# duyhominhnguyen/conan-fgw

Hardware: AMD Instinct MI355X
Metric: molecules/s (K=5 conformers) (higher is better)
Workload: dtype f32

## Files before the change

### conan-fgw_amd/csrc/fgw_common.h

```cpp
#pragma once
#include <type_traits>
#include "common.h"

#ifdef CONAN_FGW_PROFILE
static __device__ long long g_fgw_prof[32];
#define FGW_PROF_ACCESSOR(name)                                                          \
    extern "C" int name(long long *out, int reset) {                                     \
        if (out && hipMemcpyFromSymbol(out, HIP_SYMBOL(g_fgw_prof), sizeof(long long) * 32) != hipSuccess) return -2; \
        if (reset) { long long z[32] = {0}; if (hipMemcpyToSymbol(HIP_SYMBOL(g_fgw_prof), z, sizeof(z)) != hipSuccess) return -2; } \
        return 0;                                                                        \
    }
static __device__ long long g_fgw_trace[2 + 6 * 8192];
#define FGW_PROF_TRACE_ACCESSOR(name)                                                    \
    extern "C" int name(long long *out, int reset) {                                     \
        if (out && hipMemcpyFromSymbol(out, HIP_SYMBOL(g_fgw_trace), sizeof(long long) * (2 + 6 * 8192)) != hipSuccess) return -2; \
        if (reset) { long long z[2] = {0, 0}; if (hipMemcpyToSymbol(HIP_SYMBOL(g_fgw_trace), z, sizeof(z)) != hipSuccess) return -2; } \
        return 0;                                                                        \
    }
#define FGW_PROF_TRACE(tag)                                                              \
    do {                                                                                 \
        if (threadIdx.x == 0) {                                                          \
            const unsigned long long i_ = atomicAdd(reinterpret_cast<unsigned long long *>(&g_fgw_trace[0]), 1ull); \
            if (i_ < 8192) {                                                             \
                long long *r_ = &g_fgw_trace[2 + 6 * i_];                                \
// ... 59 lines not shown
    int *order;
};
template <int NT>
__device__ __forceinline__ void adj_scatter_lds_bytes(const FgwAdj &A, int g, int N, int P, unsigned char *m, int tid) {
    const int lo = A.gptr[g], n = min(A.gptr[g + 1] - lo, N);
    const int e0 = A.rowptr[lo], e1 = A.rowptr[lo + n];
    for (int e = e0 + tid; e < e1; e += NT) {
        const int i = A.tgt[e] - lo, j = A.col[e] - lo;
        if (i >= 0 && i < N && j >= 0 && j < N) {
            const unsigned o = (unsigned)(j * P + i);
            atomicAdd(reinterpret_cast<unsigned *>(m + (o & ~3u)), 1u << (8 * (o & 3u)));
        }
    }
}
template <int NT>
__device__ __forceinline__ const float *adj_dense_slice(const FgwAdj &A, int g, int N, int tid) {
    float *dst = A.dense + (size_t)g * N * N;
    for (int t = tid; t < N * N; t += NT) dst[t] = 0.f;
    __syncthreads();
    const int lo = A.gptr[g], n = min(A.gptr[g + 1] - lo, N);
    const int e0 = A.rowptr[lo], e1 = A.rowptr[lo + n];
    for (int e = e0 + tid; e < e1; e += NT) {
        const int i = A.tgt[e] - lo, j = A.col[e] - lo;
        if (i >= 0 && i < N && j >= 0 && j < N) atomicAdd(&dst[j * N + i], 1.0f);
    }
    __threadfence_block();
    __syncthreads();
    return dst;
}

struct FastConst {
    double two_alpha, one_m_alpha, four_alpha_inv_eps, inv_eps, inner_tol, stop_thr, inv_n;
};
inline FastConst fast_const(const conan_fgw_params &prm, int N) {
    const double alpha = (double)prm.alpha, inv_eps = 1.0 / (double)prm.epsilon;
    return FastConst{2.0 * alpha, 1.0 - alpha, 4.0 * alpha * inv_eps, inv_eps, (double)prm.inner_tol, (double)prm.stop_thr, 1.0 / (double)N};
}

__device__ __forceinline__ double exp_acc(double x) {
    if (x < -745.0) return 0.0;
    const double t = x * 1.4426950408889634074;
    const double n = rint(t);
    const float f = (float)(t - n);
    const float e = __builtin_amdgcn_exp2f(f);
    return ldexp((double)e, (int)n);
}

__device__ __forceinline__ double exp_fast(double x) {
    const double xc = fmin(fmax(x, -700.0), 700.0);
    const double t = xc * 1.4426950408889634074;
    const double sh = t + 6755399441055744.0;
    const int n = __double2loint(sh);
    const double f = t - (sh - 6755399441055744.0);
    const double e = (double)__builtin_amdgcn_exp2f((float)f);
    const double scale = __hiloint2double((n + 1023) << 20, 0);
    const double r = e * scale;
    return x > -700.0 ? (x < 700.0 ? r : __builtin_inf()) : 0.0;
}

__device__ __forceinline__ double rcp_pos(double s) {
    double r = __builtin_amdgcn_rcp(s);
    r = fma(fma(-s, r, 1.0), r, r);
    r = fma(fma(-s, r, 1.0), r, r);
    return r;
}

__device__ __forceinline__ double log_acc(double s) {
    const double y0 = (double)(__builtin_amdgcn_logf((float)s) * 0.693147180559945309f);
    const double r = s * exp_acc(-y0) - 1.0;
    return y0 + (r - 0.5 * r * r);
}

__device__ __forceinline__ double wave_sum_d(double v) {
#pragma unroll
    for (int o = 32; o > 0; o >>= 1) v += __shfl_xor(v, o, 64);
    return v;
}
__device__ __forceinline__ double wave_max_d(double v) {
#pragma unroll
    for (int o = 32; o > 0; o >>= 1) { double w = __shfl_xor(v, o, 64); v = w > v ? w : v; }
    return v;
}

template <int NW = FGW_WAVES>
__device__ __forceinline__ double block_sum_d(double v, double *red) {
    v = wave_sum_d(v);
    __syncthreads();
    if ((threadIdx.x & 63) == 0) red[threadIdx.x >> 6] = v;
    __syncthreads();
    double s = 0.0;
#pragma unroll
    for (int w = 0; w < NW; ++w) s += red[w];
    return s;
}


typedef double f64x4 __attribute__((ext_vector_type(4)));

__device__ __forceinline__ double exp_lse(double x) {
    const float f = (float)x;
    return (double)__builtin_amdgcn_exp2f(f * 1.44269504088896340736f);
}

template <int NW = FGW_WAVES, class FX, class FW, class FS>
__device__ __forceinline__ void mm_f64_pad(int M, int Nn, int Kd, FX X, FW W, FS st) {
    const int lane = threadIdx.x & 63, wave = __builtin_amdgcn_readfirstlane((int)(threadIdx.x >> 6));
    const int Mq = (M + 15) >> 4, Nq = (Nn + 15) >> 4;
    const int li = lane & 15, lk = lane >> 4;
    for (int t = wave; t < Mq * Nq; t += NW) {
        const int i0 = (t / Nq) << 4, j0 = (t % Nq) << 4;
        const int ia = i0 + li, jb = j0 + li;
        const bool ra = ia < M, cb = jb < Nn;
        const int ic = ra ? ia : M - 1, jc = cb ? jb : Nn - 1;
        f64x4 acc = {0.0, 0.0, 0.0, 0.0};
        int k0 = 0;
        for (; k0 + 16 <= Kd; k0 += 16) {
            double a[4], b[4];
#pragma unroll
            for (int u = 0; u < 4; ++u) { a[u] = X(ic, k0 + 4 * u + lk); b[u] = W(k0 + 4 * u + lk, jc); }
#pragma unroll
            for (int u = 0; u < 4; ++u) acc = __builtin_amdgcn_mfma_f64_16x16x4f64(ra ? a[u] : 0.0, cb ? b[u] : 0.0, acc, 0, 0, 0);
        }
        if (k0 < Kd) {
            double a[4], b[4];
#pragma unroll
            for (int u = 0; u < 4; ++u) {
                const int k = k0 + 4 * u + lk, kc = k < Kd ? k : Kd - 1;
                a[u] = X(ic, kc); b[u] = W(kc, jc);
            }
#pragma unroll
            for (int u = 0; u < 4; ++u) {
                const bool kin = k0 + 4 * u + lk < Kd;
                if (k0 + 4 * u < Kd)
                    acc = __builtin_amdgcn_mfma_f64_16x16x4f64((ra && kin) ? a[u] : 0.0, (cb && kin) ? b[u] : 0.0, acc, 0, 0, 0);
            }
        }
#pragma unroll
        for (int q = 0; q < 4; ++q) {
            const int i = i0 + lk + 4 * q;
            if (i < M && cb) st(i, jb, acc[q]);
        }
    }
}

template <int NW, bool WT, typename TX, typename TW, class FS>
__device__ __forceinline__ void mm_f64_glb(int M, int Nn, int Kd, const TX *__restrict__ X, int pX, const TW *__restrict__ W, int pW, FS st,
                                           const int tid = threadIdx.x) {
    const int lane = tid & 63, wave = __builtin_amdgcn_readfirstlane(tid >> 6);
    const int Mq = (M + 15) >> 4, Nq = (Nn + 15) >> 4;
    const int li = lane & 15, lk = lane >> 4;
    for (int t = wave; t < Mq * Nq; t += NW) {
        const int i0 = (t / Nq) << 4, j0 = (t % Nq) << 4;
        const int ia = i0 + li, jb = j0 + li;
        const bool ra = ia < M, cb = jb < Nn;
        const TX *xr = X + (size_t)(ra ? ia : M - 1) * pX;
        const int jc = cb ? jb : Nn - 1;
        f64x4 acc = {0.0, 0.0, 0.0, 0.0}, acc2 = {0.0, 0.0, 0.0, 0.0};
        for (int k0 = 0; k0 < Kd; k0 += 16) {
            const int kb = k0 + 4 * lk;
            double a[4], b[4];
            if (k0 + 16 <= Kd) {
#pragma unroll
                for (int u = 0; u < 4; ++u) a[u] = (double)xr[kb + u];
                if (WT) {
                    const TW *wr = W + (size_t)jc * pW + kb;
#pragma unroll
                    for (int u = 0; u < 4; ++u) b[u] = (double)wr[u];
                } else {
#pragma unroll
                    for (int u = 0; u < 4; ++u) b[u] = (double)W[(size_t)(kb + u) * pW + jc];
                }
// ... 756 lines not shown
```

### conan-fgw_amd/csrc/fgw_small.hip

```cpp
#include "fgw_common.h"

#ifdef CONAN_FGW_PROFILE
FGW_PROF_ACCESSOR(conan_debug_fgw_prof)
FGW_PROF_TRACE_ACCESSOR(conan_debug_fgw_trace)
#endif

namespace {

constexpr int SK_SCRATCH_DOUBLES = 3 * 256 + 2 * 64;

template <int R, bool KL, bool SECOND = false>
__global__ void __launch_bounds__(FGW_THREADS, (SECOND || R > 9) ? 1 : 3) k_fgw_coupling_small(
    const float *__restrict__ Ys, const float *__restrict__ Cs, const float *__restrict__ ps, const float *__restrict__ pb,
    FgwDims D, conan_fgw_params prm, int outer, int y_zero, const double *__restrict__ Cw, const double *__restrict__ Yw,
    const int *__restrict__ active, float *__restrict__ Tw, int *__restrict__ info, fgw_part_t *__restrict__ Ypart,
    fgw_part_t *__restrict__ Cpart, const double *__restrict__ zvec, const double *__restrict__ yvec, const int *__restrict__ only, FgwAdj adj) {
    extern __shared__ __attribute__((aligned(16))) char smem[];
    auto solve = [&](const int cid) {
    const int b = cid / D.K, s = cid % D.K;
    if (!fgw_active(active, D.B, b, outer)) return;
    const int N = D.N, P = D.P, d = D.d;
    const int NN = N * N, NP = N * P;
    const int tid = threadIdx.x, lane = tid & 63, w = __builtin_amdgcn_readfirstlane(tid >> 6);
    const bool lane_ok = lane < N;
// ... 276 lines not shown

    if (!prm.fixed_features && Ypart) {
        fgw_part_t *Yp = Ypart + ((size_t)b * D.K + s) * N * d;
        if (z_lds) {
            const int Nd = N * d;
            for (int t0 = tid; t0 < Nd; t0 += 4 * FGW_THREADS) {
                float zv[4];
#pragma unroll
                for (int u = 0; u < 4; ++u) { const int t = t0 + u * FGW_THREADS; zv[u] = Z[t < Nd ? t : Nd - 1]; }
#pragma unroll
                for (int u = 0; u < 4; ++u) { const int t = t0 + u * FGW_THREADS; if (t < Nd) Zl2[t] = zv[u]; }
            }
            __syncthreads();
            mm_lds<FGW_WAVES, false>(N, d, N, Tl, P, Zl2, d, [&](int i, int c, double v) { Yp[(size_t)i * d + c] = (fgw_part_t)v; }, border_prepare(N, d));
        } else {
            mm_f64(N, d, N, [&](int i, int k) { return (double)Tl[i * P + k]; }, [&](int k, int c) { return (double)Z[(size_t)k * d + c]; },
                   [&](int i, int c, double v) { Yp[(size_t)i * d + c] = (fgw_part_t)v; });
        }
    }
    FGW_PROF(9);
    if (!prm.fixed_structure) {
        fgw_part_t *Cp = Cpart + ((size_t)b * D.K + s) * NN;
        if constexpr (KL)
            mm_f64(N, N, N, [&](int i, int k) { return (double)Tl[i * P + k]; },
                   [&](int k, int j) { const double cv = (double)C2l[k * P + j]; return log(cv > 1e-15 ? cv : 1e-15); },
                   [&](int i, int j, double v) { Al[i * P + j] = v; }, bnn);
        else
            mm_lds<FGW_WAVES, false>(N, N, N, Tl, P, C2l, P, [&](int i, int j, double v) { Al[i * P + j] = v; }, bnn);
        __syncthreads();
        mm_lds<FGW_WAVES, true>(N, N, N, Al, P, Tl, P, [&](int i, int j, double v) { Cp[i * N + j] = (fgw_part_t)v; }, bnn);
    }
    FGW_PROF(10);
    FGW_PROF_FLUSH;
    };
    if constexpr (!SECOND) solve(blockIdx.x);
    else {
        const int total = D.B * D.K, base = (int)blockIdx.x * 64, l = (int)threadIdx.x & 63;
        unsigned long long m = __ballot(base + l < total && only[base + l < total ? base + l : 0] != 0);
        while (m) {
            const int k = __ffsll((long long)m) - 1;
            m &= m - 1;
            solve(base + k);
            __syncthreads();
        }
    }
}

template <int R> struct FastCfg {
    static constexpr int OCC = R <= 9 ? 5 : (R <= 12 ? 2 : 1);
};
inline int fast_tiles_per_wave(int N) {
    const int Mc = (N >> 4) << 4;
    const bool border = (N - Mc) * N + Mc * (N - Mc) <= FGW_WAVES * 32 && Mc > 0;
    const int q = border ? N >> 4 : (N + 15) >> 4;
    return (q * q + FGW_WAVES - 1) / FGW_WAVES;
}
constexpr int FAST_VEC_DOUBLES = 128 + 256;
constexpr int FAST_SK_DOUBLES = 2 * 256 + 2 * 64;

struct FastLds {
    int npa;
    size_t off_t, off_c2, off_red, off_vec, off_sk, off_rs, bytes;
    bool vec_alias, sk_alias;
};
template <typename C2T>
__host__ __device__ inline FastLds fast_lds(int N) {
    FastLds L;
    const int NP = N * fgw_pitch(N);
    L.npa = (NP + 1) & ~1;
    size_t o = (size_t)3 * L.npa * 8;
    L.off_t = o; o += ((size_t)NP * 4 + 15) & ~(size_t)15;
    L.off_c2 = o; o += ((size_t)NP * sizeof(C2T) + 15) & ~(size_t)15;
    L.off_red = o; o += 64;
    L.vec_alias = (size_t)NP * 4 >= FAST_VEC_DOUBLES * 8;
    L.sk_alias = L.npa >= FAST_SK_DOUBLES;
    L.off_vec = L.vec_alias ? L.off_t : o; if (!L.vec_alias) o += FAST_VEC_DOUBLES * 8;
    L.off_sk = L.sk_alias ? (size_t)L.npa * 8 : o; if (!L.sk_alias) o += FAST_SK_DOUBLES * 8;
    const bool rs_alias = (size_t)NP * sizeof(C2T) >= (size_t)4 * N * 8;
    L.off_rs = rs_alias ? L.off_c2 : o; if (!rs_alias) o += (size_t)4 * N * 8;
    L.bytes = o;
    return L;
}

template <int R, int MAXT, typename C2T>
__global__ void __launch_bounds__(FGW_THREADS, FastCfg<R>::OCC) k_fgw_coupling_fast(
    const float *__restrict__ Ys, const float *__restrict__ Cs, const float *__restrict__ ps, const float *__restrict__ pb,
    FgwDims D, conan_fgw_params prm, FastConst fc, int outer, int y_zero, const double *__restrict__ Cw, const double *__restrict__ Yw,
    const int *__restrict__ active, float *__restrict__ Tw, int *__restrict__ info, fgw_part_t *__restrict__ Ypart,
    fgw_part_t *__restrict__ Cpart, const double *__restrict__ zvec, const double *__restrict__ yvec, int *__restrict__ redo, FgwAdj adj) {
    extern __shared__ __attribute__((aligned(16))) char smem[];
    int cid = (gridDim.x & 7) == 0 ? xcd_contiguous_block((int)blockIdx.x, (int)gridDim.x) : (int)blockIdx.x;
    if (adj.order && (gridDim.x & 7) == 0) {
        const int x = (int)blockIdx.x & 7, pblk = (int)blockIdx.x >> 3;
        cid = adj.order[x + 8 * (pblk / D.K)] * D.K + pblk % D.K;
    }
    const int b = cid / D.K, s = cid % D.K;
    if (!fgw_active(active, D.B, b, outer)) return;
    const int N = D.N, P = D.P, d = D.d;
    const int NN = N * N;
    const int tid = threadIdx.x, lane = tid & 63, w = __builtin_amdgcn_readfirstlane(tid >> 6);
    FGW_PROF_DECL;

    const FastLds L = fast_lds<C2T>(N);
    double *C1l = reinterpret_cast<double *>(smem);
    double *AKl = C1l + L.npa;
    double *Bl = AKl + L.npa;
    float *Tl = reinterpret_cast<float *>(smem + L.off_t);
    C2T *C2l = reinterpret_cast<C2T *>(smem + L.off_c2);
    double *red = reinterpret_cast<double *>(smem + L.off_red);
    float *t_dummy = reinterpret_cast<float *>(red + 7);
    double *pq = reinterpret_cast<double *>(smem + L.off_vec);
    double *vec4 = pq + 128;
    double *bufC = reinterpret_cast<double *>(smem + L.off_sk);
    double *bufR = bufC + 256;
    double *fvP = bufR + 256;
    double *gvP = fvP + 64;
    double *Yl = AKl;
    float *Zl = reinterpret_cast<float *>(C1l);
    const bool yz_lds = d <= 2 * P;

    const float *Z = Ys + ((size_t)b * D.K + s) * N * d;
    const float *C2 = Cs + ((size_t)b * D.K + s) * NN;
    const double *C1 = Cw + (size_t)b * NN;
    const double *Y = Yw + (size_t)b * N * d;
    float *Tg = Tw + ((size_t)b * D.K + s) * NN;

    constexpr int EPT = (16 * R * R + FGW_THREADS - 1) / FGW_THREADS;
    const int e_dq = FGW_THREADS / N, e_dr = FGW_THREADS - e_dq * N;
    const int e_i0 = tid / N, e_j0 = tid - e_i0 * N;
    auto for_entries = [&](auto fn) {
        int i = e_i0, j = e_j0;
#pragma unroll
        for (int u = 0; u < EPT; ++u) {
            if (tid + u * FGW_THREADS < NN) fn(u, i * P + j);
            j += e_dr; i += e_dq;
            if (j >= N) { j -= N; ++i; }
        }
    };
    const bool warm = outer > 0 && prm.warmstart;
    const bool stage_yz = d <= 2 * P && !y_zero;
    const bool ragged = sizeof(C2T) == 1 && adj.rowptr != nullptr;
    float c2v[EPT];
#pragma unroll
    for (int u = 0; u < EPT; ++u) { const int t = tid + u * FGW_THREADS; c2v[u] = ragged ? 0.f : C2[t < NN ? t : NN - 1]; }
    double c1v[EPT];
    float tv[EPT];
    auto load_c1_t = [&]() {
#pragma unroll
        for (int u = 0; u < EPT; ++u) {
            const int t = tid + u * FGW_THREADS, tc = t < NN ? t : NN - 1;
            c1v[u] = C1[tc]; tv[u] = warm ? Tg[tc] : 0.f;
        }
    };
    if (!stage_yz) load_c1_t();
    const double p_own = tid < N ? (pb ? (double)pb[(size_t)b * N + tid] : fc.inv_n) : 1.0;
    const double q_own = tid < N ? (ps ? (double)ps[((size_t)b * D.K + s) * N + tid] : fc.inv_n) : 1.0;
    double vec_own;
    {
        const int v = tid >> 6, i = tid & 63;
        const double *src = (v == 0 || v == 2) ? yvec + (size_t)b * 2 * N + (v == 0 ? N : 0) : zvec + ((size_t)b * D.K + s) * 2 * N + (v == 1 ? N : 0);
        vec_own = src[i < N ? i : N - 1];
        vec_own = i < N ? vec_own : 0.0;
    }
    int nb = N;
    if (ragged) nb = min(adj.gptr[cid + 1] - adj.gptr[cid], N);
    const bool pad_try = !pb && !ps && !Ypart && !prm.fixed_structure && !prm.fixed_features;
    auto c1_block_ok = [&](int nb_) {
        auto near = [](double a, double b_) { return fabs(a - b_) <= 1e-9 * (fabs(b_) + 1e-30) || a == b_; };
        bool ok = true;
        const int lc = lane < N ? lane : N - 1;
        const double c_nb = C1[(size_t)nb_ * N + lc];
        const double cbb = __shfl(c_nb, nb_, 64);
        const double want = lane < nb_ ? c_nb : cbb;
        for (int r = nb_ + 1 + w; r < N; r += FGW_WAVES) ok = ok && (lane >= N || near(C1[(size_t)r * N + lc], want));
        ok = ok && (lane < nb_ || lane >= N || near(c_nb, cbb));
        const int mcol = N - nb_;
        for (int k = w; k < nb_; k += FGW_WAVES) {
            const double v = C1[(size_t)k * N + nb_ + (lane < mcol ? lane : 0)];
            ok = ok && near(v, __shfl(v, 0, 64));
        }
        return ok;
    };
    bool pad_ok = pad_try && ragged && N - nb >= 2 && nb >= 1;
    if (pad_ok) pad_ok = c1_block_ok(nb);
    if (stage_yz) {
        const int Nd = N * d;
        for (int t0 = tid; t0 < Nd; t0 += 4 * FGW_THREADS) {
            double yv[4]; float zv[4];
#pragma unroll
            for (int u = 0; u < 4; ++u) { const int t = t0 + u * FGW_THREADS, tc = t < Nd ? t : Nd - 1; yv[u] = Y[tc]; zv[u] = Z[tc]; }
#pragma unroll
            for (int u = 0; u < 4; ++u) { const int t = t0 + u * FGW_THREADS; if (t < Nd) { Yl[t] = yv[u]; Zl[t] = zv[u]; } }
        }
    }
    if (tid < 64) { pq[tid] = p_own; pq[64 + tid] = q_own; }
    vec4[tid] = vec_own;
    for_entries([&](int u, int o) { C2l[o] = (C2T)c2v[u]; if (!stage_yz) C1l[o] = c1v[u]; });
    if constexpr (sizeof(C2T) == 1) {
        if (ragged) {
            __syncthreads();
            adj_scatter_lds_bytes<FGW_THREADS>(adj, cid, N, P, reinterpret_cast<unsigned char *>(C2l), tid);
        }
    }
    __syncthreads();
    int n_real;
    {
        const bool nz = lane < N && C2l[lane] != (C2T)0;
        n_real = 1 + __popcll(__ballot(nz));
    }
    bool complete;
    {
        bool ok = true;
        int i = e_i0, j = e_j0;
#pragma unroll
        for (int u = 0; u < EPT; ++u) {
            if (tid + u * FGW_THREADS < NN) ok = ok && (C2l[i * P + j] == (C2T)((i != j && i < n_real && j < n_real) ? 1 : 0));
            j += e_dr; i += e_dq;
            if (j >= N) { j -= N; ++i; }
        }
        complete = __syncthreads_and(ok) != 0 && n_real >= 2;
    }
    double *rsum = reinterpret_cast<double *>(smem + L.off_rs);
    if (!ragged) {
        int mx = 1;
        int i = e_i0, j = e_j0;
#pragma unroll
        for (int u = 0; u < EPT; ++u) {
            if (tid + u * FGW_THREADS < NN && C2l[i * P + j] != (C2T)0) mx = max(mx, max(i, j) + 1);
            j += e_dr; i += e_dq;
            if (j >= N) { j -= N; ++i; }
        }
#pragma unroll
        for (int o = 32; o > 0; o >>= 1) mx = max(mx, __shfl_xor(mx, o, 64));
        int *ired = reinterpret_cast<int *>(red);
        if (lane == 0) ired[w] = mx;
        __syncthreads();
        nb = max(max(ired[0], ired[1]), max(ired[2], ired[3]));
        __syncthreads();
        pad_ok = pad_try && N - nb >= 2 && nb >= 1;
        if (pad_ok) pad_ok = c1_block_ok(nb);
    }
    int m_pad = 0;
    if (pad_try && N - nb >= 2 && nb >= 1) {
        auto nearf = [](double a, double b_) { return fabs(a - b_) <= 1e-9 * (fabs(b_) + 1e-30) || a == b_; };
        bool ok = pad_ok;
        for (int r = nb + 1 + w; r < N; r += FGW_WAVES)
            for (int c = lane; c < d; c += 64) {
                if (stage_yz) {
                    ok = ok && nearf((double)Zl[r * d + c], (double)Zl[nb * d + c]) && nearf(Yl[r * d + c], Yl[nb * d + c]);
                } else {
                    ok = ok && nearf((double)Z[(size_t)r * d + c], (double)Z[(size_t)nb * d + c]);
                    if (!y_zero) ok = ok && nearf(Y[(size_t)r * d + c], Y[(size_t)nb * d + c]);
                }
            }
        if (__syncthreads_and(ok) != 0) m_pad = N - nb;
    }
    const int Nx = m_pad ? nb + 1 : N;
    const double mult = m_pad ? (double)m_pad : 1.0;
    FGW_PROF(0);
    const double qj = pq[64 + lane] * ((m_pad && lane == nb) ? mult : 1.0);
    const double pi_l = pq[lane] * ((m_pad && lane == nb) ? mult : 1.0);
    const double *r1v = vec4, *r2v = vec4 + 64, *y2v = vec4 + 128, *z2v = vec4 + 192;
    auto base_of = [&](int i, int j, double dot) {
        double m = -2.0 * dot; m += y2v[i]; m += z2v[j];
        m = m > 0.0 ? m : 0.0;
        return fc.two_alpha * (r1v[i] + r2v[j]) + fc.one_m_alpha * m;
    };
    if (y_zero) {
        int i = e_i0, j = e_j0;
#pragma unroll
        for (int u = 0; u < EPT; ++u) {
            if (tid + u * FGW_THREADS < NN) Bl[i * P + j] = base_of(i, j, 0.0);
            j += e_dr; i += e_dq;
            if (j >= N) { j -= N; ++i; }
        }
    } else if (stage_yz) {
        mm_lds2<FGW_WAVES, MAXT, 0, true, true>(Nx, Nx, d, Yl, d, Zl, d, [&]() { load_c1_t(); __syncthreads(); },
                                                [&](int i, int j, double v) { Bl[i * P + j] = base_of(i, j, v); });
        for_entries([&](int u, int o) { C1l[o] = c1v[u]; });
    } else {
        mm_f64(Nx, Nx, d, [&](int i, int k) { return Y[(size_t)i * d + k]; }, [&](int k, int j) { return (double)Z[(size_t)j * d + k]; },
               [&](int i, int j, double v) { Bl[i * P + j] = base_of(i, j, v); });
    }
    __syncthreads();
    FGW_PROF(1);
    if (warm) {
        if (m_pad) {
            int i = e_i0, j = e_j0;
#pragma unroll
            for (int u = 0; u < EPT; ++u) {
                if (tid + u * FGW_THREADS < NN) Tl[i * P + j] = (float)((double)tv[u] * ((i == nb ? mult : 1.0) * (j == nb ? mult : 1.0)));
                j += e_dr; i += e_dq;
                if (j >= N) { j -= N; ++i; }
            }
        } else {
            for_entries([&](int u, int o) { Tl[o] = tv[u]; });
        }
    } else {
#pragma unroll
        for (int r = 0; r < R; ++r) {
            const int i = w + 4 * r;
            const double pi_r = (pb ? (double)pb[(size_t)b * N + (i < N ? i : N - 1)] : fc.inv_n) * ((m_pad && i == nb) ? mult : 1.0);
            if (i < Nx && lane < Nx) Tl[i * P + lane] = (float)(pi_r * qj);
        }
    }
    __syncthreads();
    FGW_PROF(2);

    int cpt = 0, sk_total = 0;
    double err = 1.0;
    bool bail = __syncthreads_or(tid < N && (p_own <= 0.0 || q_own <= 0.0)) != 0;
    while (!bail && err > fc.inner_tol && cpt < prm.max_iter) {
        int tq = tid, N = Nx, P = D.P;
        asm volatile("" : "+v"(tq), "+s"(N), "+s"(P));
        int nbq = m_pad ? nb : -1;
        asm volatile("" : "+s"(nbq));
        const int lq = tq & 63, wq = tq >> 6;
        const bool lq_ok = lq < N;
        mm_lds2<FGW_WAVES, 1, 0, false, false>(N, N, N, C1l, P, Tl, P, [] {}, [&](int i, int j, double v) { AKl[i * P + j] = v; }, tq);
        __syncthreads();
        FGW_PROF(3);
        int nr = n_real;
        asm volatile("" : "+s"(nr));
        if (complete) {
            {
                const int lc = lq_ok ? lq : N - 1;
                const double *ar = AKl + lc * P + wq;
                double p0 = 0.0, p1 = 0.0;
#pragma unroll
                for (int r = 0; r < R; ++r) {
                    const int q = wq + 4 * r;
                    if (q < nr) { if (r & 1) p1 += ar[4 * r]; else p0 += ar[4 * r]; }
                }
                if (lq_ok) rsum[wq * N + lq] = p0 + p1;
            }
            __syncthreads();
            {
                int i = tq / N, j = tq - i * N;
                const int dq = FGW_THREADS / N, dr = FGW_THREADS - dq * N;
                for (int t = tq; t < N * N; t += FGW_THREADS) {
                    const int o = i * P + j;
                    const double ai = ((rsum[i] + rsum[N + i]) + rsum[2 * N + i]) + rsum[3 * N + i];
                    const double v = j < nr ? ai - AKl[o] : 0.0;
                    const double x = fma(v, fc.four_alpha_inv_eps, (Bl[j * P + j] - Bl[o]) * fc.inv_eps);
                    AKl[o] = exp_fast(x);
                    j += dr; i += dq;
                    if (j >= N) { j -= N; ++i; }
                }
            }
        } else {
            mm_lds2<FGW_WAVES, MAXT, 0, true, true>(N, N, N, AKl, P, C2l, P, [&]() { __syncthreads(); }, [&](int i, int j, double v) {
                const double x = fma(v, fc.four_alpha_inv_eps, (Bl[j * P + j] - Bl[i * P + j]) * fc.inv_eps);
                AKl[i * P + j] = exp_fast(x);
            }, tq);
        }
        __syncthreads();
        FGW_PROF(4);
        double kA[R], kB[R];
        {
            const int lc = lq_ok ? lq : N - 1;
#pragma unroll
            for (int r = 0; r < R; ++r) {
                const int q = wq + 4 * r, qc = q < N ? q : N - 1;
                const double a = AKl[qc * P + lc], bb = AKl[lc * P + qc];
                const bool ok = q < N && lq_ok;
                kA[r] = ok ? a : 0.0; kB[r] = ok ? bb : 0.0;
            }
        }
        __syncthreads();
        FGW_PROF(5);
        const int permL = (lq & 3) * 16 + (lq >> 2);
        double *bufCw = bufC + wq * 64 + lq, *bufRw = bufR + wq * 64 + lq;
        const double *fw = fvP + wq * 16, *gw = gvP + wq * 16;
        auto dotR = [&](const double (&k)[R], const double *v) {
            double p0 = 0.0, p1 = 0.0, p2 = 0.0;
#pragma unroll
            for (int r = 0; r < R; ++r) {
                if (r % 3 == 0) p0 = fma(k[r], v[r], p0);
                else if (r % 3 == 1) p1 = fma(k[r], v[r], p1);
                else p2 = fma(k[r], v[r], p2);
            }
            return (p0 + p1) + p2;
        };
        int ii = 0;
        double f = 0.0, g = 0.0, colp = 0.0;
        bool have_colp = false;
        for (; ii < prm.num_iter_max; ++ii) {
            if (!have_colp) {
                double pc = 0.0;
                if (ii == 0) {
                    gvP[permL] = lq_ok ? (lq == nbq ? (double)m_pad : 1.0) : 0.0;
                }
                pc = dotR(kA, gw);
                *bufCw = pc;
                __syncthreads();
                colp = ((bufC[lq] + bufC[64 + lq]) + bufC[128 + lq]) + bufC[192 + lq];
            }
            have_colp = false;
            if (__any(lq_ok && !(colp > 1e-150 && colp < 1e150))) { bail = true; break; }
            f = lq_ok ? qj * rcp_pos(colp) : 0.0;
            fvP[permL] = f;
            *bufRw = dotR(kB, fw);
            __syncthreads();
            const double rs = ((bufR[lq] + bufR[64 + lq]) + bufR[128 + lq]) + bufR[192 + lq];
            if (__any(lq_ok && !(rs > 1e-150 && rs < 1e150))) { bail = true; break; }
            g = lq_ok ? pi_l * rcp_pos(rs) : 0.0;
            gvP[permL] = g;
            if (ii % 10 == 0) {
                *bufCw = dotR(kA, gw);
                __syncthreads();
                colp = ((bufC[lq] + bufC[64 + lq]) + bufC[128 + lq]) + bufC[192 + lq];
                have_colp = true;
                double df = lq_ok ? f * colp - qj : 0.0;
                df = df * df;
                if (lq == nbq) df /= (double)m_pad;
                df = wave_sum_d(df);
                if (sqrt(df) < fc.stop_thr) { ++ii; break; }
            }
        }
        if (bail) break;
        sk_total += ii;
        FGW_PROF(6);
        double e2 = 0.0;
        {
            float *trow = Tl + wq * P + lq;
#pragma unroll
            for (int r = 0; r < R; ++r) {
                const bool ok = lq_ok && wq + 4 * r < N;
                float *tp = ok ? trow + 4 * r * P : t_dummy;
                const float tn = (float)((gw[r] * kA[r]) * f);
                double df = ok ? (double)tn - (double)*tp : 0.0;
                df *= df;
                if (nbq >= 0) {
                    const double im = 1.0 / (double)m_pad;
                    df *= (lq == nbq ? im : 1.0) * (wq + 4 * r == nbq ? im : 1.0);
                }
                e2 += df;
                *tp = tn;
            }
        }
        if (cpt % 10 == 0) err = sqrt(block_sum_d(e2, red));
        else __syncthreads();
        ++cpt;
        FGW_PROF(7);
    }
    if (bail) {
        if (tid == 0) { redo[cid] = 1; atomicOr(&info[b * 4 + 3], 1); }
        return;
    }
    __syncthreads();
    {
        int te = tid;
        asm volatile("" : "+v"(te));
        int i = te / N, j = te - i * N;
        const int dq = FGW_THREADS / N, dr = FGW_THREADS - dq * N;
        if (m_pad) {
            const float im = (float)(1.0 / mult);
            for (int t = te; t < NN; t += FGW_THREADS) {
                Tg[t] = Tl[min(i, nb) * P + min(j, nb)] * ((i >= nb ? im : 1.0f) * (j >= nb ? im : 1.0f));
                j += dr; i += dq;
                if (j >= N) { j -= N; ++i; }
            }
        } else {
            for (int t = te; t < NN; t += FGW_THREADS) {
                Tg[t] = Tl[i * P + j];
                j += dr; i += dq;
                if (j >= N) { j -= N; ++i; }
            }
        }
    }
    if (tid == 0) { atomicAdd(&info[b * 4 + 1], cpt); atomicAdd(&info[b * 4 + 2], sk_total); redo[cid] = 0; if (m_pad) atomicOr(&info[b * 4 + 3], 2); }
    FGW_PROF(8);

    if (!prm.fixed_features && Ypart) {
        fgw_part_t *Yp = Ypart + ((size_t)b * D.K + s) * N * d;
        if (yz_lds) {
            const int Nd = N * d;
            for (int t0 = tid; t0 < Nd; t0 += 4 * FGW_THREADS) {
                float zv[4];
#pragma unroll
                for (int u = 0; u < 4; ++u) { const int t = t0 + u * FGW_THREADS; zv[u] = Z[t < Nd ? t : Nd - 1]; }
#pragma unroll
                for (int u = 0; u < 4; ++u) { const int t = t0 + u * FGW_THREADS; if (t < Nd) Zl[t] = zv[u]; }
            }
            __syncthreads();
            mm_lds2<FGW_WAVES, 1, 0, false, false>(N, d, N, Tl, P, Zl, d, [] {}, [&](int i, int c, double v) { Yp[(size_t)i * d + c] = (fgw_part_t)v; });
        } else {
            mm_f64(N, d, N, [&](int i, int k) { return (double)Tl[i * P + k]; }, [&](int k, int c) { return (double)Z[(size_t)k * d + c]; },
                   [&](int i, int c, double v) { Yp[(size_t)i * d + c] = (fgw_part_t)v; });
        }
    }
    FGW_PROF(9);
    if (!prm.fixed_structure) {
        fgw_part_t *Cp = Cpart + ((size_t)b * D.K + s) * NN;
        if (complete) {
            {
                const int lc = lane < Nx ? lane : Nx - 1;
                const float *tr = Tl + lc * P + w;
                double p0 = 0.0, p1 = 0.0;
#pragma unroll
                for (int r = 0; r < R; ++r) {
                    const int q = w + 4 * r;
                    if (q < n_real) { if (r & 1) p1 += (double)tr[4 * r]; else p0 += (double)tr[4 * r]; }
                }
                if (lane < Nx) rsum[w * N + lane] = p0 + p1;
            }
            __syncthreads();
            mm_lds2<FGW_WAVES, 1, 0, true, false>(Nx, Nx, n_real, Tl, P, Tl, P, [] {}, [&](int i, int j, double v) {
                const double ti = ((rsum[i] + rsum[N + i]) + rsum[2 * N + i]) + rsum[3 * N + i];
                const double tj = ((rsum[j] + rsum[N + j]) + rsum[2 * N + j]) + rsum[3 * N + j];
                if (m_pad) Bl[i * P + j] = ti * tj - v;
                else Cp[i * N + j] = (fgw_part_t)(ti * tj - v);
            });
        } else {
            mm_lds2<FGW_WAVES, 1, 0, false, false>(Nx, Nx, Nx, Tl, P, C2l, P, [] {}, [&](int i, int j, double v) { AKl[i * P + j] = v; });
            __syncthreads();
            mm_lds2<FGW_WAVES, 1, 0, true, false>(Nx, Nx, Nx, AKl, P, Tl, P, [] {}, [&](int i, int j, double v) {
                if (m_pad) Bl[i * P + j] = v;
                else Cp[i * N + j] = (fgw_part_t)v;
            });
        }
        if (m_pad) {
            __syncthreads();
            const double im = 1.0 / mult;
            int i = tid / N, j = tid - i * N;
            const int dq = FGW_THREADS / N, dr = FGW_THREADS - dq * N;
            for (int t = tid; t < NN; t += FGW_THREADS) {
                Cp[t] = (fgw_part_t)(Bl[min(i, nb) * P + min(j, nb)] * ((i >= nb ? im : 1.0) * (j >= nb ? im : 1.0)));
                j += dr; i += dq;
                if (j >= N) { j -= N; ++i; }
            }
        }
    }
    FGW_PROF(10);
    FGW_PROF_FLUSH;
    FGW_PROF_TRACE(Nx | (cpt << 8) | (sk_total << 20));
}

template <int NT>
__device__ __forceinline__ void molecule_vectors(const double *__restrict__ Y, const double *__restrict__ C, const float *__restrict__ p, int N,
                                                 int d, bool kl, double *__restrict__ out, int which = 2) {
    constexpr int LPI = NT / 64;
    const int i = (int)threadIdx.x / LPI, sub = (int)threadIdx.x % LPI;
    double y2 = 0.0, r1 = 0.0;
    if (i < N) {
        if (which != 1)
            for (int c = sub; c < d; c += LPI) { const double v = Y[(size_t)i * d + c]; y2 += v * v; }
        if (which != 0)
            for (int k = sub; k < N; k += LPI) {
                const double c1 = C[i * N + k], pk = p ? (double)p[k] : 1.0 / (double)N;
                r1 += (kl ? c1 * log(c1 + 1e-15) - c1 : c1 * c1) * pk;
            }
    }
#pragma unroll
    for (int o = 1; o < LPI; o <<= 1) { y2 += __shfl_xor(y2, o, 64); r1 += __shfl_xor(r1, o, 64); }
    if (i < N && sub == 0) { if (which != 1) out[i] = y2; if (which != 0) out[N + i] = r1; }
}

__global__ void __launch_bounds__(256) k_fgw_small_vectors(const float *__restrict__ Ys, const float *__restrict__ Cs, const float *__restrict__ ps,
                                                           const float *__restrict__ pb, FgwDims D, int kl, double *__restrict__ Cw,
                                                           double *__restrict__ Yw, double *__restrict__ zvec, double *__restrict__ yvec,
                                                           const float *__restrict__ init_C, const float *__restrict__ init_Y, int max_iter,
                                                           int *__restrict__ active, int *__restrict__ info, float *__restrict__ errs,
                                                           float *__restrict__ Yout, float *__restrict__ Cout, FgwAdj adj) {
    const int b = blockIdx.x / D.K, s = blockIdx.x % D.K;
    const int N = D.N, d = D.d;
    __shared__ __attribute__((aligned(16))) unsigned char cm[64 * 65 + 16];
    const int Pm = D.P;
    if (adj.rowptr) {
        for (int t = threadIdx.x; t < (64 * 65 + 16) / 4; t += 256) reinterpret_cast<unsigned *>(cm)[t] = 0u;
        __syncthreads();
        adj_scatter_lds_bytes<256>(adj, (int)blockIdx.x, N, Pm, cm, (int)threadIdx.x);
        __syncthreads();
    }
    if (s == 0) {
        const int NN = N * N, Nd = N * d;
        const float *c0 = init_C ? init_C + (size_t)b * NN : Cs + (size_t)b * D.K * NN;
        for (int t = threadIdx.x; t < NN; t += 256) {
            const float cv = (!init_C && adj.rowptr) ? (float)cm[(t / N) * Pm + (t % N)] : c0[t];
            Cw[(size_t)b * NN + t] = (double)cv; Cout[(size_t)b * NN + t] = cv;
        }
        for (int t = threadIdx.x; t < Nd; t += 256) {
            const float y = init_Y ? init_Y[(size_t)b * Nd + t] : 0.f;
            Yw[(size_t)b * Nd + t] = (double)y; Yout[(size_t)b * Nd + t] = y;
        }
        if (threadIdx.x == 0) { fgw_active_init(active, D.B, b); info[b * 4 + 0] = 0; info[b * 4 + 1] = 0; info[b * 4 + 2] = 0; info[b * 4 + 3] = 0; }
        for (int t = threadIdx.x; t < 2 * max_iter; t += 256) errs[(size_t)b * 2 * max_iter + t] = __builtin_nanf("");
        __syncthreads();
    }
    const float *Z = Ys + ((size_t)b * D.K + s) * N * d;
    const float *C2 = Cs + ((size_t)b * D.K + s) * N * N;
    const float *q = ps ? ps + ((size_t)b * D.K + s) * N : nullptr;
    const int j = (int)threadIdx.x >> 2, sub = (int)threadIdx.x & 3;
    double z2 = 0.0, r2 = 0.0;
    if (j < N) {
        for (int c = sub; c < d; c += 4) { const double v = (double)Z[(size_t)j * d + c]; z2 += v * v; }
        for (int k = sub; k < N; k += 4) {
            const double c2 = adj.rowptr ? (double)cm[j * Pm + k] : (double)C2[j * N + k], qk = q ? (double)q[k] : 1.0 / (double)N;
            r2 += qk * (kl ? c2 : c2 * c2);
        }
    }
    z2 += __shfl_xor(z2, 1, 64); z2 += __shfl_xor(z2, 2, 64);
    r2 += __shfl_xor(r2, 1, 64); r2 += __shfl_xor(r2, 2, 64);
    double *zo = zvec + ((size_t)b * D.K + s) * 2 * N;
    if (j < N && sub == 0) { zo[j] = z2; zo[N + j] = r2; }
    if (s == 0)
        molecule_vectors<256>(Yw + (size_t)b * N * d, Cw + (size_t)b * N * N, pb ? pb + (size_t)b * N : nullptr, N, d, kl != 0, yvec + (size_t)b * 2 * N);
    if (adj.order && blockIdx.x == gridDim.x - 1) fgw_order_by_size<256>(adj, D.B, D.K, (int)threadIdx.x);
}

// ... 102 lines not shown
                    }
#pragma unroll
                    for (int u = 0; u < U; ++u) {
                        const int t = t0 + u * UPD_THREADS;
                        if (t < Nd) {
                            const double df = acc[u] - old[u];
                            e2 += df * df;
                            Yb[t] = acc[u];
                            Yout[(size_t)b * Nd + t] = (float)acc[u];
                        }
                    }
                }
            }
        }
    } else if (!prm.fixed_structure) {
        double *Cb = Cw + (size_t)b * NN;
        for (int t0 = tid; t0 < NN; t0 += U * UPD_THREADS) {
            double acc[U], old[U];
#pragma unroll
            for (int u = 0; u < U; ++u) {
                const int t = t0 + u * UPD_THREADS;
                acc[u] = 0.0; old[u] = 0.0;
                if (t < NN) {
                    old[u] = Cb[t];
                    for (int s = 0; s < K; ++s) {
                        const double lam = lambdas ? (double)lambdas[s] : 1.0 / (double)K;
                        acc[u] += lam * Cpart[((size_t)b * K + s) * NN + t];
                    }
                }
            }
#pragma unroll
            for (int u = 0; u < U; ++u) {
                const int t = t0 + u * UPD_THREADS;
                if (t < NN) {
                    const int i = t / N, j = t - i * N;
                    const double pi = pb ? (double)pb[(size_t)b * N + i] : 1.0 / (double)N;
                    const double pj = pb ? (double)pb[(size_t)b * N + j] : 1.0 / (double)N;
                    const double cn = pi * pj > 0.0 ? (prm.loss_fun ? exp(acc[u] / (pi * pj)) : acc[u] / (pi * pj)) : 0.0;
                    const double df = cn - old[u];
                    e2 += df * df;
                    Cb[t] = cn;
                    Cout[(size_t)b * NN + t] = (float)cn;
                }
            }
        }
    }
    const double err = sqrt(block_sum_d<UPD_THREADS / 64>(e2, red));
    if (yvec) molecule_vectors<UPD_THREADS>(Yw + (size_t)b * Nd, Cw + (size_t)b * NN, pb ? pb + (size_t)b * N : nullptr, N, d, prm.loss_fun != 0,
                                            yvec + (size_t)b * 2 * N, part);
    if (tid == 0) {
        errs[((size_t)b * 2 + part) * prm.max_iter + outer] = (float)err;
        info[b * 4 + 0] = outer + 1;
        *flag_out = err > (double)prm.tol ? 1 : 0;
    }
}

inline size_t small_lds(int N, int d) {
    const size_t NP = (size_t)N * fgw_pitch(N);
    (void)d; return NP * 8 * 4 + (256 + 128 + 8 + (NP >= (size_t)SK_SCRATCH_DOUBLES ? 0 : SK_SCRATCH_DOUBLES)) * 8 + NP * 4 * 2;
}

}

bool conan_fgw_small_supported(int N, int d) { return N <= 64 && small_lds(N, d) <= 160 * 1024; }

void conan_fgw_small_prepare(const FgwCall &c) {
    k_fgw_small_vectors<<<c.D.B * c.D.K, 256, 0, c.s>>>(c.Ys, c.Cs, c.ps, c.p, c.D, c.prm.loss_fun, c.Cw, c.Yw, c.zvec, c.yvec, c.init_C, c.init_Y,
                                                       c.prm.max_iter, c.active, c.info, c.errs, c.Y, c.C, c.adj);
}

template <class F>
static void with_rows(int R, F &&f) {
    if (R <= 6) f(std::integral_constant<int, 6>{});
    else if (R <= 9) f(std::integral_constant<int, 9>{});
    else if (R <= 12) f(std::integral_constant<int, 12>{});
    else f(std::integral_constant<int, 16>{});
}

template <int R, typename C2T>
static void launch_fast(const FgwCall &c, int outer, int y_zero, fgw_part_t *Ypart) {
    const FgwDims &D = c.D;
    const int tpw = fast_tiles_per_wave(D.N);
    auto go = [&](auto kernel) {
        launch_lds(kernel, D.B * D.K, FGW_THREADS, fast_lds<C2T>(D.N).bytes, c.s, c.Ys, c.Cs, c.ps, c.p, D, c.prm, fast_const(c.prm, D.N), outer,
                   y_zero, c.Cw, c.Yw, c.active, c.T, c.info, Ypart, c.Cpart, c.zvec, c.yvec, c.redo, c.adj);
    };
    if constexpr (R <= 6) go(k_fgw_coupling_fast<R, 1, C2T>);
    else if constexpr (R <= 12) { if (tpw <= 1) go(k_fgw_coupling_fast<R, 1, C2T>); else go(k_fgw_coupling_fast<R, 3, C2T>); }
    else { if (tpw <= 1) go(k_fgw_coupling_fast<R, 1, C2T>); else if (tpw <= 3) go(k_fgw_coupling_fast<R, 3, C2T>); else go(k_fgw_coupling_fast<R, 4, C2T>); }
}

bool conan_fgw_fast_supported(int N, int d, int small_int) {
    if (N > 64 || N < 4) return false;
    const size_t lds = small_int ? fast_lds<unsigned char>(N).bytes : fast_lds<float>(N).bytes;
    return lds <= 160 * 1024 && d >= 1;
}

void conan_fgw_small_coupling(const FgwCall &c, int outer, int y_zero, fgw_part_t *Ypart) {
    const FgwDims &D = c.D;
    const size_t lds = small_lds(D.N, D.d);
    const int grid = D.B * D.K;
    const bool kl = c.prm.loss_fun != 0;
    with_rows((D.N + 3) / 4, [&](auto R) {
        const int *only = nullptr;
        if (!kl && conan_fgw_fast_supported(D.N, D.d, c.prm.cs_small_int)) {
            if (c.prm.cs_small_int) launch_fast<R.value, unsigned char>(c, outer, y_zero, Ypart);
            else launch_fast<R.value, float>(c, outer, y_zero, Ypart);
            only = c.redo;
        }
        auto exact = [&](auto kernel, int blocks) {
            launch_lds(kernel, blocks, FGW_THREADS, lds, c.s, c.Ys, c.Cs, c.ps, c.p, D, c.prm, outer, y_zero, c.Cw, c.Yw, c.active, c.T, c.info, Ypart,
                       c.Cpart, c.zvec, c.yvec, only, c.adj);
        };
        if (kl) exact(k_fgw_coupling_small<R.value, true, false>, grid);
        else if (only) exact(k_fgw_coupling_small<R.value, false, true>, (grid + 63) / 64);
        else exact(k_fgw_coupling_small<R.value, false, false>, grid);
    });
}

void conan_fgw_small_update(const FgwCall &c, int outer, bool y_from_t) {
    const FgwDims &D = c.D;
    const int chunk = y_from_t ? conan_fgw_update_chunk(D.K, D.N, D.d, D.B) : 0;
    if (chunk > 0)
        launch_lds(k_fgw_update_parts<true>, 2 * D.B, UPD_THREADS, (size_t)chunk * ((size_t)D.N * D.N + (size_t)D.N * D.d) * 4, c.s, c.p, c.lambdas, D,
                   c.prm, outer, nullptr, c.Cpart, c.Cw, c.Yw, c.active, c.info, c.errs, c.Y, c.C, c.yvec, c.T, c.Ys, chunk);
    else
        k_fgw_update_parts<false><<<2 * D.B, UPD_THREADS, 0, c.s>>>(c.p, c.lambdas, D, c.prm, outer, c.Ypart, c.Cpart, c.Cw, c.Yw, c.active, c.info, c.errs,
                                                                     c.Y, c.C, c.yvec, nullptr, nullptr, 0);
}

int conan_fgw_update_chunk(int K, int N, int d, int B) {
    if (N > 64) return 0;
    const size_t per = ((size_t)N * N + (size_t)N * d) * 4, budget = (2 * B <= 256 ? 144 : 72) * 1024;
    if (per > budget) return 0;
    const int c = (int)(budget / per);
    return c < K ? c : K;
}
```

Before: 116,700.

## Reload epilogue pointers from kernarg and use ds_swizzle wave reductions

```diff
diff --git a/conan-fgw_amd/csrc/fgw_common.h b/conan-fgw_amd/csrc/fgw_common.h
--- a/conan-fgw_amd/csrc/fgw_common.h
+++ b/conan-fgw_amd/csrc/fgw_common.h
@@ -165,11 +165,23 @@
     return v;
 }
 
-template <int NW = FGW_WAVES>
-__device__ __forceinline__ double block_sum_d(double v, double *red) {
-    v = wave_sum_d(v);
+template <int O>
+__device__ __forceinline__ double swizzle_xor_d(double v) {
+    static_assert(O > 0 && O < 32, "ds_swizzle's bit mode works within 32 lanes");
+    const int lo = __builtin_amdgcn_ds_swizzle(__double2loint(v), (O << 10) | 0x1f), hi = __builtin_amdgcn_ds_swizzle(__double2hiint(v), (O << 10) | 0x1f);
+    return __hiloint2double(hi, lo);
+}
+__device__ __forceinline__ double wave_sum_d_lean(double v) {
+    v += __shfl_xor(v, 32, 64);
+    v += swizzle_xor_d<16>(v); v += swizzle_xor_d<8>(v); v += swizzle_xor_d<4>(v); v += swizzle_xor_d<2>(v); v += swizzle_xor_d<1>(v);
+    return v;
+}
+
+template <int NW = FGW_WAVES, bool LEAN = false>
+__device__ __forceinline__ double block_sum_d(double v, double *red, const int tid = threadIdx.x) {
+    v = LEAN ? wave_sum_d_lean(v) : wave_sum_d(v);
     __syncthreads();
-    if ((threadIdx.x & 63) == 0) red[threadIdx.x >> 6] = v;
+    if ((tid & 63) == 0) red[tid >> 6] = v;
     __syncthreads();
     double s = 0.0;
 #pragma unroll
diff --git a/conan-fgw_amd/csrc/fgw_small.hip b/conan-fgw_amd/csrc/fgw_small.hip
--- a/conan-fgw_amd/csrc/fgw_small.hip
+++ b/conan-fgw_amd/csrc/fgw_small.hip
@@ -382,13 +382,25 @@
     return L;
 }
 
+struct FastTail {
+    const float *Ys;
+    float *Tw;
+    int *info;
+    fgw_part_t *Ypart, *Cpart;
+    int *redo;
+    int K;
+};
+typedef const FastTail __attribute__((address_space(4))) *FastTailPtr;
+
 template <int R, int MAXT, typename C2T>
 __global__ void __launch_bounds__(FGW_THREADS, FastCfg<R>::OCC) k_fgw_coupling_fast(
-    const float *__restrict__ Ys, const float *__restrict__ Cs, const float *__restrict__ ps, const float *__restrict__ pb,
+    FastTail tail, const float *__restrict__ Cs, const float *__restrict__ ps, const float *__restrict__ pb,
     FgwDims D, conan_fgw_params prm, FastConst fc, int outer, int y_zero, const double *__restrict__ Cw, const double *__restrict__ Yw,
-    const int *__restrict__ active, float *__restrict__ Tw, int *__restrict__ info, fgw_part_t *__restrict__ Ypart,
-    fgw_part_t *__restrict__ Cpart, const double *__restrict__ zvec, const double *__restrict__ yvec, int *__restrict__ redo, FgwAdj adj) {
+    const int *__restrict__ active, const double *__restrict__ zvec, const double *__restrict__ yvec, FgwAdj adj) {
     extern __shared__ __attribute__((aligned(16))) char smem[];
+    const float *__restrict__ Ys = tail.Ys;
+    const float *__restrict__ Tw = tail.Tw;
+    const bool y_parts = tail.Ypart != nullptr;
     int cid = (gridDim.x & 7) == 0 ? xcd_contiguous_block((int)blockIdx.x, (int)gridDim.x) : (int)blockIdx.x;
     if (adj.order && (gridDim.x & 7) == 0) {
         const int x = (int)blockIdx.x & 7, pblk = (int)blockIdx.x >> 3;
@@ -423,7 +435,7 @@
     const float *C2 = Cs + ((size_t)b * D.K + s) * NN;
     const double *C1 = Cw + (size_t)b * NN;
     const double *Y = Yw + (size_t)b * N * d;
-    float *Tg = Tw + ((size_t)b * D.K + s) * NN;
+    const float *Tg = Tw + ((size_t)b * D.K + s) * NN;
 
     constexpr int EPT = (16 * R * R + FGW_THREADS - 1) / FGW_THREADS;
     const int e_dq = FGW_THREADS / N, e_dr = FGW_THREADS - e_dq * N;
@@ -464,7 +476,7 @@
     }
     int nb = N;
     if (ragged) nb = min(adj.gptr[cid + 1] - adj.gptr[cid], N);
-    const bool pad_try = !pb && !ps && !Ypart && !prm.fixed_structure && !prm.fixed_features;
+    const bool pad_try = !pb && !ps && !y_parts && !prm.fixed_structure && !prm.fixed_features;
     auto c1_block_ok = [&](int nb_) {
         auto near = [](double a, double b_) { return fabs(a - b_) <= 1e-9 * (fabs(b_) + 1e-30) || a == b_; };
         bool ok = true;
@@ -613,8 +625,8 @@
     while (!bail && err > fc.inner_tol && cpt < prm.max_iter) {
         int tq = tid, N = Nx, P = D.P;
         asm volatile("" : "+v"(tq), "+s"(N), "+s"(P));
-        int nbq = m_pad ? nb : -1;
-        asm volatile("" : "+s"(nbq));
+        int nbq = m_pad ? nb : -1, mq = m_pad;
+        asm volatile("" : "+s"(nbq), "+s"(mq));
         const int lq = tq & 63, wq = tq >> 6;
         const bool lq_ok = lq < N;
         mm_lds2<FGW_WAVES, 1, 0, false, false>(N, N, N, C1l, P, Tl, P, [] {}, [&](int i, int j, double v) { AKl[i * P + j] = v; }, tq);
@@ -689,7 +701,7 @@
             if (!have_colp) {
                 double pc = 0.0;
                 if (ii == 0) {
-                    gvP[permL] = lq_ok ? (lq == nbq ? (double)m_pad : 1.0) : 0.0;
+                    gvP[permL] = lq_ok ? (lq == nbq ? (double)mq : 1.0) : 0.0;
                 }
                 pc = dotR(kA, gw);
                 *bufCw = pc;
@@ -713,8 +725,8 @@
                 have_colp = true;
                 double df = lq_ok ? f * colp - qj : 0.0;
                 df = df * df;
-                if (lq == nbq) df /= (double)m_pad;
-                df = wave_sum_d(df);
+                if (lq == nbq) df /= (double)mq;
+                df = wave_sum_d_lean(df);
                 if (sqrt(df) < fc.stop_thr) { ++ii; break; }
             }
         }
@@ -732,30 +744,38 @@
                 double df = ok ? (double)tn - (double)*tp : 0.0;
                 df *= df;
                 if (nbq >= 0) {
-                    const double im = 1.0 / (double)m_pad;
+                    const double im = 1.0 / (double)mq;
                     df *= (lq == nbq ? im : 1.0) * (wq + 4 * r == nbq ? im : 1.0);
                 }
                 e2 += df;
                 *tp = tn;
             }
         }
-        if (cpt % 10 == 0) err = sqrt(block_sum_d(e2, red));
+        if (cpt % 10 == 0) err = sqrt(block_sum_d<FGW_WAVES, true>(e2, red, tq));
         else __syncthreads();
         ++cpt;
         FGW_PROF(7);
     }
+    FastTailPtr tl = (FastTailPtr)__builtin_amdgcn_kernarg_segment_ptr();
+    asm volatile("" : "+s"(tl));
+    int *info = tl->info, *redo = tl->redo;
     if (bail) {
         if (tid == 0) { redo[cid] = 1; atomicOr(&info[b * 4 + 3], 1); }
         return;
     }
     __syncthreads();
+    auto fresh_tid = [&]() { int t = tid; asm volatile("" : "+v"(t)); return t; };
+    int te = fresh_tid();
+    int me = m_pad;
+    asm volatile("" : "+s"(me));
+    const double mult_e = me ? (double)me : 1.0;
+    const size_t cs = (size_t)b * tl->K + s;
     {
-        int te = tid;
-        asm volatile("" : "+v"(te));
+        float *Tg = tl->Tw + cs * NN;
         int i = te / N, j = te - i * N;
         const int dq = FGW_THREADS / N, dr = FGW_THREADS - dq * N;
         if (m_pad) {
-            const float im = (float)(1.0 / mult);
+            const float im = (float)(1.0 / mult_e);
             for (int t = te; t < NN; t += FGW_THREADS) {
                 Tg[t] = Tl[min(i, nb) * P + min(j, nb)] * ((i >= nb ? im : 1.0f) * (j >= nb ? im : 1.0f));
                 j += dr; i += dq;
@@ -769,14 +789,16 @@
             }
         }
     }
-    if (tid == 0) { atomicAdd(&info[b * 4 + 1], cpt); atomicAdd(&info[b * 4 + 2], sk_total); redo[cid] = 0; if (m_pad) atomicOr(&info[b * 4 + 3], 2); }
+    if (te == 0) { atomicAdd(&info[b * 4 + 1], cpt); atomicAdd(&info[b * 4 + 2], sk_total); redo[cid] = 0; if (m_pad) atomicOr(&info[b * 4 + 3], 2); }
     FGW_PROF(8);
-
-    if (!prm.fixed_features && Ypart) {
-        fgw_part_t *Yp = Ypart + ((size_t)b * D.K + s) * N * d;
+    te = fresh_tid();
+
+    if (!prm.fixed_features && tl->Ypart) {
+        fgw_part_t *Yp = tl->Ypart + cs * N * d;
+        const float *Z = tl->Ys + cs * N * d;
         if (yz_lds) {
             const int Nd = N * d;
-            for (int t0 = tid; t0 < Nd; t0 += 4 * FGW_THREADS) {
+            for (int t0 = te; t0 < Nd; t0 += 4 * FGW_THREADS) {
                 float zv[4];
 #pragma unroll
                 for (int u = 0; u < 4; ++u) { const int t = t0 + u * FGW_THREADS; zv[u] = Z[t < Nd ? t : Nd - 1]; }
@@ -784,7 +806,7 @@
                 for (int u = 0; u < 4; ++u) { const int t = t0 + u * FGW_THREADS; if (t < Nd) Zl[t] = zv[u]; }
             }
             __syncthreads();
-            mm_lds2<FGW_WAVES, 1, 0, false, false>(N, d, N, Tl, P, Zl, d, [] {}, [&](int i, int c, double v) { Yp[(size_t)i * d + c] = (fgw_part_t)v; });
+            mm_lds2<FGW_WAVES, 1, 0, false, false>(N, d, N, Tl, P, Zl, d, [] {}, [&](int i, int c, double v) { Yp[(size_t)i * d + c] = (fgw_part_t)v; }, te);
         } else {
             mm_f64(N, d, N, [&](int i, int k) { return (double)Tl[i * P + k]; }, [&](int k, int c) { return (double)Z[(size_t)k * d + c]; },
                    [&](int i, int c, double v) { Yp[(size_t)i * d + c] = (fgw_part_t)v; });
@@ -792,40 +814,45 @@
     }
     FGW_PROF(9);
     if (!prm.fixed_structure) {
-        fgw_part_t *Cp = Cpart + ((size_t)b * D.K + s) * NN;
+        fgw_part_t *Cp = tl->Cpart + cs * NN;
+        te = fresh_tid();
         if (complete) {
             {
-                const int lc = lane < Nx ? lane : Nx - 1;
-                const float *tr = Tl + lc * P + w;
+                const int le = te & 63, we = __builtin_amdgcn_readfirstlane(te >> 6);
+                const int lc = le < Nx ? le : Nx - 1;
+                const float *tr = Tl + lc * P + we;
                 double p0 = 0.0, p1 = 0.0;
 #pragma unroll
                 for (int r = 0; r < R; ++r) {
-                    const int q = w + 4 * r;
+                    const int q = we + 4 * r;
                     if (q < n_real) { if (r & 1) p1 += (double)tr[4 * r]; else p0 += (double)tr[4 * r]; }
                 }
-                if (lane < Nx) rsum[w * N + lane] = p0 + p1;
+                if (le < Nx) rsum[we * N + le] = p0 + p1;
             }
             __syncthreads();
+            te = fresh_tid();
             mm_lds2<FGW_WAVES, 1, 0, true, false>(Nx, Nx, n_real, Tl, P, Tl, P, [] {}, [&](int i, int j, double v) {
                 const double ti = ((rsum[i] + rsum[N + i]) + rsum[2 * N + i]) + rsum[3 * N + i];
                 const double tj = ((rsum[j] + rsum[N + j]) + rsum[2 * N + j]) + rsum[3 * N + j];
                 if (m_pad) Bl[i * P + j] = ti * tj - v;
                 else Cp[i * N + j] = (fgw_part_t)(ti * tj - v);
-            });
+            }, te);
         } else {
-            mm_lds2<FGW_WAVES, 1, 0, false, false>(Nx, Nx, Nx, Tl, P, C2l, P, [] {}, [&](int i, int j, double v) { AKl[i * P + j] = v; });
+            mm_lds2<FGW_WAVES, 1, 0, false, false>(Nx, Nx, Nx, Tl, P, C2l, P, [] {}, [&](int i, int j, double v) { AKl[i * P + j] = v; }, te);
             __syncthreads();
+            te = fresh_tid();
             mm_lds2<FGW_WAVES, 1, 0, true, false>(Nx, Nx, Nx, AKl, P, Tl, P, [] {}, [&](int i, int j, double v) {
                 if (m_pad) Bl[i * P + j] = v;
                 else Cp[i * N + j] = (fgw_part_t)v;
-            });
+            }, te);
         }
         if (m_pad) {
             __syncthreads();
-            const double im = 1.0 / mult;
-            int i = tid / N, j = tid - i * N;
+            const double im = 1.0 / mult_e;
+            te = fresh_tid();
+            int i = te / N, j = te - i * N;
             const int dq = FGW_THREADS / N, dr = FGW_THREADS - dq * N;
-            for (int t = tid; t < NN; t += FGW_THREADS) {
+            for (int t = te; t < NN; t += FGW_THREADS) {
                 Cp[t] = (fgw_part_t)(Bl[min(i, nb) * P + min(j, nb)] * ((i >= nb ? im : 1.0) * (j >= nb ? im : 1.0)));
                 j += dr; i += dq;
                 if (j >= N) { j -= N; ++i; }
@@ -1094,8 +1121,8 @@
     const FgwDims &D = c.D;
     const int tpw = fast_tiles_per_wave(D.N);
     auto go = [&](auto kernel) {
-        launch_lds(kernel, D.B * D.K, FGW_THREADS, fast_lds<C2T>(D.N).bytes, c.s, c.Ys, c.Cs, c.ps, c.p, D, c.prm, fast_const(c.prm, D.N), outer,
-                   y_zero, c.Cw, c.Yw, c.active, c.T, c.info, Ypart, c.Cpart, c.zvec, c.yvec, c.redo, c.adj);
+        launch_lds(kernel, D.B * D.K, FGW_THREADS, fast_lds<C2T>(D.N).bytes, c.s, FastTail{c.Ys, c.T, c.info, Ypart, c.Cpart, c.redo, D.K}, c.Cs, c.ps,
+                   c.p, D, c.prm, fast_const(c.prm, D.N), outer, y_zero, c.Cw, c.Yw, c.active, c.zvec, c.yvec, c.adj);
     };
     if constexpr (R <= 6) go(k_fgw_coupling_fast<R, 1, C2T>);
     else if constexpr (R <= 12) { if (tpw <= 1) go(k_fgw_coupling_fast<R, 1, C2T>); else go(k_fgw_coupling_fast<R, 3, C2T>); }
```

Result: no change. 117,200 (median of 6 runs) (+0.4%).
